# Kr-Stam/CUDA_Optical_Flow_2

Measured on AMD Instinct MI355X. Metric: Mpix/s dense LK flow, higher is better.
Workload: dtype i32/f64; 1 GPU; 3840x2160 pair, 5-level pyramid, 9x9 window, iters=5 (BASELINE.json config as written; iterations = extension lk_iter: bilinear-warp refinement, iteration 1 = the reference bit for bit), mode lk_float, stream path: new frame's pyramid + every LK level and iteration, inputs resident in HBM; SURVEY 8d's smooth texture translating by (2,1) px per frame; warmup_steps_run=5

## Files before the change

### cuda_optical_flow_2_amd/csrc/lk_body_pair.h

```cpp
#pragma once

namespace ofx_dev {

template <int R>
struct TileGeomP {
    static constexpr int FIRST_COL = 2 * R + 2;
    static constexpr int LO_LANE = (FIRST_COL + 3) / 4;
    static constexpr int HI_LANE = 63 - LO_LANE;
    static constexpr int OUT_W = (HI_LANE - LO_LANE + 1) * 4;
    static_assert(4 * LO_LANE >= FIRST_COL && 4 * HI_LANE + 3 <= 253 - 2 * R, "B's output columns have all of A's results they need");
};
static_assert(TileGeomP<4>::LO_LANE == 3 && TileGeomP<4>::HI_LANE == 60 && TileGeomP<4>::OUT_W == 232, "9x9: lanes 3..60");
static_assert(TileGeomP<3>::LO_LANE == 2 && TileGeomP<3>::HI_LANE == 61 && TileGeomP<3>::OUT_W == 240, "7x7: lanes 2..61");
static_assert(TileGeomP<2>::LO_LANE == 2 && TileGeomP<2>::HI_LANE == 61 && TileGeomP<2>::OUT_W == 240, "5x5: lanes 2..61");
static_assert(TileGeomP<1>::LO_LANE == 1 && TileGeomP<1>::HI_LANE == 62 && TileGeomP<1>::OUT_W == 248, "3x3: lanes 1..62");

constexpr int kLkPairMaxR = 4;
constexpr int pair_warp_rows(int r) { return 2 * r + 4; }
constexpr int pair_flow_rows(int r) { return r + 3; }
constexpr int pair_wave_lds(int r) { return kLkWaveLds + 256 * pair_warp_rows(r) + 2048 * pair_flow_rows(r); }
static_assert(pair_wave_lds(4) == 19584 && 8 * pair_wave_lds(4) <= 160 * 1024, "two waves per SIMD at 9x9");

constexpr int pair_seg_steps(int r) { return 3 * r + 4; }

template <int R, bool FAST, bool INTERIOR, bool WOUT>
__device__ __forceinline__ void lk_wave_pair(const LkTable &T, int level, int tile, int ysB, int yeB, int lane, uint8_t *xlds, int q1, int q2, int q3)
{
    constexpr int MODE = OFX_MODE_LK_FLOAT;
    using G = TileGeomP<R>;
    constexpr int NS = 2 * R + 1, H = R - 1, PR = 2 * R - H;
    constexpr int kLagSteps = 2 * R + 3;
    constexpr int WN = pair_warp_rows(R), FN = pair_flow_rows(R);
    static_assert(PR + kLagSteps == pair_seg_steps(R), "a segment of r rows takes r + 3R + 4 steps");

    LkArgs A = T.lv[level];
    pin_scalar(A.w);
    pin_scalar(A.h);
    pin_scalar(A.pitch);
    pin_scalar(A.min_det);
    pin_scalar(A.warp_scale);
    const SolveOpts sopt{A.min_det};
    const int cb = tile * G::OUT_W - G::LO_LANE * 4 + 4 * lane;
    const int ysA = ysB - (R + 1), yeA = min(yeB + R + 1, A.h);

    const int plane_bytes = A.h * A.pitch;
    const __amdgpu_buffer_rsrc_t rs_prev = make_rsrc(A.prev, plane_bytes), rs_next = make_rsrc(A.next, plane_bytes);
    const __amdgpu_buffer_rsrc_t rs_fin = make_rsrc(A.flow_in, A.h * A.w * 8), rs_flow = make_rsrc(A.flow, A.h * A.w * 8);
    const __amdgpu_buffer_rsrc_t rs_wsrc = make_rsrc(A.warp_src, plane_bytes + 3);
    [[maybe_unused]] __amdgpu_buffer_rsrc_t rs_wout = rs_prev;
    if constexpr (WOUT) rs_wout = make_rsrc(A.warp_out, plane_bytes);

    const bool ld_ok = INTERIOR || (cb >= 0 && cb < A.w);
    uint32_t bmask = INTERIOR ? 0xffffffffu : 0u;
    if constexpr (!INTERIOR) {
#pragma unroll
        for (int j = 0; j < 4; ++j) {
            const bool in = (cb + j) >= 0 && (cb + j) < A.w;
            bmask |= in ? (0xffu << (8 * j)) : 0u;
        }
    }
    uint32_t col_off = ld_ok ? (uint32_t)cb : 0u;
    uint32_t nat_off = (uint32_t)cb * 8u;
    auto finish_row = [&](uint32_t raw) -> uint32_t {
        if constexpr (INTERIOR) return raw;
        else return raw & bmask;
    };
    const int x0 = tile * G::OUT_W;
    const int nv = min(x0 + G::OUT_W, A.w) - x0;
    uint32_t l16 = 16u * (uint32_t)lane;
    const int lim = 8 * nv - 16, c16 = 16 * lane;
    const bool st_lo4 = c16 <= lim, st_lo2 = c16 == lim + 8, st_hi4 = c16 <= lim - 1024, st_hi2 = c16 == lim + 8 - 1024;
    const uint32_t vo_lo = st_lo4 ? l16 : (uint32_t)kOob, vo_hi = st_hi4 ? l16 + 1024u : (uint32_t)kOob;
    const bool ragged = __any(st_lo2 || st_hi2) != 0;
    const lds_ptr xl_w = (lds_ptr)xlds + 32 * lane;
    const lds_ptr xl_base = (lds_ptr)xlds + 32 * G::LO_LANE;
    const lds_ptr wring = (lds_ptr)xlds + kLkWaveLds + 4 * lane;
    const lds_ptr fring = (lds_ptr)xlds + kLkWaveLds + 256 * WN + 32 * lane;
    auto wslot = [&](int y) -> int { return __builtin_amdgcn_readfirstlane((int)((uint32_t)(y + 2 * WN) % (uint32_t)WN) * 256); };
    auto fslot = [&](int y) -> int { return __builtin_amdgcn_readfirstlane((int)((uint32_t)(y + 4 * FN) % (uint32_t)FN) * 2048); };
    [[maybe_unused]] uint32_t wvo = (uint32_t)kOob;
    if constexpr (WOUT) {
        const bool out_lane = lane >= G::LO_LANE && lane <= G::HI_LANE && cb < A.w;
        wvo = out_lane ? (uint32_t)cb : (uint32_t)kOob;
    }
    uint32_t wmiss = 0u;
    WarpRowState WA;
    [[maybe_unused]] WarpRowState WB;
    warp_row_clear(WA);
    if constexpr (WOUT) warp_row_clear(WB);
    const s2 two = pk_two();
    const int fstep = A.w * 8;

    const int y_limA = min(yeA + R + 1, A.h);
    const int y_firstA = ysA - R, y_lo0A = y_firstA + H;
    const int nstepsA = (yeA - ysA) + PR;
    const int y_min_outA = max(0, y_firstA - 1), span_outA = max(y_limA - y_min_outA, 0);
    auto row_offA = [&](int y) -> int { return (uint32_t)y < (uint32_t)y_limA ? y * A.pitch : kOob; };
    auto row_off_outA = [&](int y) -> int { return (uint32_t)(y - y_min_outA) < (uint32_t)span_outA ? y * A.pitch : kOob; };
    auto load_u32 = [&](const __amdgpu_buffer_rsrc_t &rs, int po) -> uint32_t { return __builtin_amdgcn_raw_buffer_load_b32(rs, col_off, po, 0); };
    RowPk<MODE> wa[3];
    {
        uint32_t pi, ni, po = 0u, no = 0u;
#pragma unroll
        for (int t = 0; t < 3; ++t) {
            const int oi = row_offA(y_lo0A - 1 + t);
            pi = finish_row(load_u32(rs_prev, oi)), ni = finish_row(load_u32(rs_next, oi));
            if constexpr (H > 0) {
                const int oo = row_off_outA(y_firstA - 1 + t);
                po = finish_row(load_u32(rs_prev, oo)), no = finish_row(load_u32(rs_next, oo));
            }
            unpack_pk(pi, ni, po, no, wa[t]);
        }
    }
    int axx[4] = {0, 0, 0, 0}, ayy[4] = {0, 0, 0, 0}, axy[4] = {0, 0, 0, 0}, axt[4] = {0, 0, 0, 0}, ayt[4] = {0, 0, 0, 0};

    auto ring_warped = [&](int y) {
        const uint32_t wn = finish_row(warp_row_finish(WA));
        *(__attribute__((address_space(3))) uint32_t *)(wring + wslot(y)) = wn;
    };
    auto stepA = [&](auto K, int s) {
        constexpr int k = decltype(K)::value;
        const int yy = y_lo0A + s, yo = yy - NS;
        const bool folded = H > 0 && s < H;
        const int yh = folded ? y_firstA + s : yo;
        const int ro = (H > 1 && s + 1 < H) ? y_firstA + s + 2 : yo + 2;
        const int po_in = row_offA(yy + 2), po_out = row_off_outA(ro);
        const uint32_t pf_ip = load_u32(rs_prev, po_in), pf_in = load_u32(rs_next, po_in);
        const uint32_t pf_op = load_u32(rs_prev, po_out), pf_on = load_u32(rs_next, po_out);
        const bool emit = s >= PR;
        const int yw = yy - R;
        f32x4 old_a, old_b;
        asm("" : "=v"(old_a), "=v"(old_b));
        if (emit) {
            const int fnat = __builtin_amdgcn_readfirstlane(yw >= 0 ? yw * fstep : kOob);
            if constexpr (INTERIOR) {
                old_a = __builtin_bit_cast(f32x4, __builtin_amdgcn_raw_buffer_load_b128(rs_fin, nat_off, fnat, 0));
                old_b = __builtin_bit_cast(f32x4, __builtin_amdgcn_raw_buffer_load_b128(rs_fin, nat_off + 16u, fnat, 0));
            } else {
                auto off = [&](int j) { return ((bmask >> (8 * j)) & 1u) ? nat_off + 8u * (uint32_t)j : (uint32_t)kOob; };
                const u32x2 p0 = __builtin_amdgcn_raw_buffer_load_b64(rs_fin, off(0), fnat, 0), p1 = __builtin_amdgcn_raw_buffer_load_b64(rs_fin, off(1), fnat, 0);
                const u32x2 p2 = __builtin_amdgcn_raw_buffer_load_b64(rs_fin, off(2), fnat, 0), p3 = __builtin_amdgcn_raw_buffer_load_b64(rs_fin, off(3), fnat, 0);
                old_a = __builtin_bit_cast(f32x4, u32x4{p0.x, p0.y, p1.x, p1.y});
                old_b = __builtin_bit_cast(f32x4, u32x4{p2.x, p2.y, p3.x, p3.y});
            }
        }
        const uint32_t him = folded ? 0x00010000u : (yo >= y_firstA ? 0xffff0000u : 0u);
        uint32_t rowm = ((uint32_t)yy < (uint32_t)A.h ? 0x00000001u : 0u) | ((uint32_t)yh < (uint32_t)A.h ? him : 0u);
        if constexpr (INTERIOR) rowm = (uint32_t)__builtin_amdgcn_readfirstlane((int)rowm);
        uint32_t mm[4];
#pragma unroll
        for (int j = 0; j < 4; ++j) mm[j] = INTERIOR ? rowm : ((uint32_t)__builtin_amdgcn_sbfe((int)bmask, 8 * j, 1) & rowm);
        s2 ix[4], iy[4], it[4];
        derivs_pk(wa[k], wa[(k + 1) % 3], wa[(k + 2) % 3], two, ix, iy, it);
        accumulate_pk(ix, iy, it, mm, axx, ayy, axy, axt, ayt);
        if (emit) {
            float uv[8];
            int hb[5][4];
            {
                int va[5][4];
#pragma unroll
                for (int j = 0; j < 4; ++j) va[0][j] = axx[j], va[1][j] = ayy[j], va[2][j] = axy[j], va[3][j] = axt[j], va[4][j] = ayt[j];
                hbox4x5<R>(va, hb);
            }
            solve_lane<MODE, FAST>(hb[0], hb[1], hb[2], hb[3], hb[4], sopt, uv);
            uv[0] = old_a.x + uv[0], uv[1] = old_a.y + uv[1], uv[2] = old_a.z + uv[2], uv[3] = old_a.w + uv[3];
            uv[4] = old_b.x + uv[4], uv[5] = old_b.y + uv[5], uv[6] = old_b.z + uv[6], uv[7] = old_b.w + uv[7];
            ring_warped(yw - 1);
            const float fu[4] = {uv[0], uv[2], uv[4], uv[6]}, fv[4] = {uv[1], uv[3], uv[5], uv[7]};
            warp_row_prepare<false>(rs_wsrc, A.warp_scale, A.w, A.h, A.pitch, 0, A.h, cb, yw, 4, fu, fv, WA, wmiss);
            const lds_ptr fr = fring + fslot(yw);
            *(__attribute__((address_space(3))) f32x4 *)(fr) = f32x4{uv[0], uv[1], uv[2], uv[3]};
            *(__attribute__((address_space(3))) f32x4 *)(fr + 16) = f32x4{uv[4], uv[5], uv[6], uv[7]};
        }
        unpack_pk(finish_row(pf_ip), finish_row(pf_in), finish_row(pf_op), finish_row(pf_on), wa[k]);
        pin_row(wa[k]);
    };

    const int y_limB = min(yeB + R + 1, A.h);
    const int y_firstB = ysB - R, y_lo0B = y_firstB + H;
    const int nstepsB = (yeB - ysB) + PR;
    const int y_min_outB = max(0, y_firstB - 1), span_outB = max(y_limB - y_min_outB, 0);
    auto row_offB = [&](int y) -> int { return (uint32_t)y < (uint32_t)y_limB ? y * A.pitch : kOob; };
    auto row_off_outB = [&](int y) -> int { return (uint32_t)(y - y_min_outB) < (uint32_t)span_outB ? y * A.pitch : kOob; };
    auto ring_row = [&](int y, int po) -> uint32_t {
        uint32_t v = 0u;
        if (po != kOob) v = *(const __attribute__((address_space(3))) uint32_t *)(wring + wslot(y));
        return v;
    };
    RowPk<MODE> wb[3];
    uint32_t pfb_i = 0u, pfb_o = 0u;
    int bxx[4] = {0, 0, 0, 0}, byy[4] = {0, 0, 0, 0}, bxy[4] = {0, 0, 0, 0}, bxt[4] = {0, 0, 0, 0}, byt[4] = {0, 0, 0, 0};
    const int fso0 = __builtin_amdgcn_readfirstlane((ysB * A.w + x0) * 8);
    auto high_rowB = [&](int s) -> int { return (H > 0 && (s == 0 || s < H)) ? y_firstB + s + 1 : y_lo0B + s - NS + 1; };
    auto primeB = [&]() {
        uint32_t pi, ni, po = 0u, no = 0u;
#pragma unroll
        for (int t = 0; t < 2; ++t) {
            const int yi = y_lo0B - 1 + t, oi = row_offB(yi);
            pi = finish_row(load_u32(rs_prev, oi)), ni = ring_row(yi, oi);
            if constexpr (H > 0) {
                const int yo = y_firstB - 1 + t, oo = row_off_outB(yo);
                po = finish_row(load_u32(rs_prev, oo)), no = ring_row(yo, oo);
            }
            unpack_pk(pi, ni, po, no, wb[t]);
        }
        pfb_i = load_u32(rs_prev, row_offB(y_lo0B + 1));
        pfb_o = load_u32(rs_prev, H > 0 ? row_off_outB(high_rowB(0)) : kOob);
    };
    auto store_row = [&](int s_row, const f32x4 xlo, const f32x4 xhi) {
        const int fso = __builtin_amdgcn_readfirstlane(fso0 + (s_row - PR) * fstep);
        __builtin_amdgcn_raw_buffer_store_b128(__builtin_bit_cast(u32x4, xlo), rs_flow, INTERIOR ? lane_off_var(l16) : vo_lo, fso, kLkStoreAux);
        __builtin_amdgcn_raw_buffer_store_b128(__builtin_bit_cast(u32x4, xhi), rs_flow, vo_hi, fso, kLkStoreAux);
        if (__builtin_expect(ragged, 0)) {
            const u32x4 ql = __builtin_bit_cast(u32x4, xlo), qh = __builtin_bit_cast(u32x4, xhi);
            __builtin_amdgcn_raw_buffer_store_b64(u32x2{ql.x, ql.y}, rs_flow, st_lo2 ? l16 : (uint32_t)kOob, fso, kLkStoreAux);
            __builtin_amdgcn_raw_buffer_store_b64(u32x2{qh.x, qh.y}, rs_flow, st_hi2 ? l16 + 1024u : (uint32_t)kOob, fso, kLkStoreAux);
        }
    };
    auto stepB = [&](auto K, int s) {
        constexpr int k = decltype(K)::value;
        const int yy = y_lo0B + s, yo = yy - NS;
        const bool folded = H > 0 && s < H;
        const int yh = folded ? y_firstB + s : yo;
        {
            const int rh = high_rowB(s);
            const int oi = row_offB(yy + 1), oo = (H > 0 || s > 0) ? row_off_outB(rh) : kOob;
            unpack_pk(finish_row(pfb_i), ring_row(yy + 1, oi), finish_row(pfb_o), ring_row(rh, oo), wb[(k + 2) % 3]);
            pin_row(wb[(k + 2) % 3]);
            pfb_i = load_u32(rs_prev, row_offB(yy + 2));
            pfb_o = load_u32(rs_prev, row_off_outB(high_rowB(s + 1)));
        }
        const bool emit = s >= PR;
        const int yw = yy - R;
        f32x4 old_a, old_b;
        asm("" : "=v"(old_a), "=v"(old_b));
        if (emit) {
            const lds_ptr fr = fring + fslot(yw);
            old_a = *(const __attribute__((address_space(3))) f32x4 *)(fr);
            old_b = *(const __attribute__((address_space(3))) f32x4 *)(fr + 16);
        }
        const uint32_t him = folded ? 0x00010000u : (yo >= y_firstB ? 0xffff0000u : 0u);
        uint32_t rowm = ((uint32_t)yy < (uint32_t)A.h ? 0x00000001u : 0u) | ((uint32_t)yh < (uint32_t)A.h ? him : 0u);
        if constexpr (INTERIOR) rowm = (uint32_t)__builtin_amdgcn_readfirstlane((int)rowm);
        uint32_t mm[4];
#pragma unroll
        for (int j = 0; j < 4; ++j) mm[j] = INTERIOR ? rowm : ((uint32_t)__builtin_amdgcn_sbfe((int)bmask, 8 * j, 1) & rowm);
        s2 ix[4], iy[4], it[4];
        derivs_pk(wb[k], wb[(k + 1) % 3], wb[(k + 2) % 3], two, ix, iy, it);
        accumulate_pk(ix, iy, it, mm, bxx, byy, bxy, bxt, byt);
        if (emit) {
            float uv[8];
            int hb[5][4];
            {
                int va[5][4];
#pragma unroll
                for (int j = 0; j < 4; ++j) va[0][j] = bxx[j], va[1][j] = byy[j], va[2][j] = bxy[j], va[3][j] = bxt[j], va[4][j] = byt[j];
                hbox4x5<R>(va, hb);
            }
            solve_lane<MODE, FAST>(hb[0], hb[1], hb[2], hb[3], hb[4], sopt, uv);
            uv[0] = old_a.x + uv[0], uv[1] = old_a.y + uv[1], uv[2] = old_a.z + uv[2], uv[3] = old_a.w + uv[3];
            uv[4] = old_b.x + uv[4], uv[5] = old_b.y + uv[5], uv[6] = old_b.z + uv[6], uv[7] = old_b.w + uv[7];
            if constexpr (WOUT) {
                const uint32_t wn = warp_row_finish(WB);
                const int wso = __builtin_amdgcn_readfirstlane(s > PR ? (yw - 1) * A.pitch : kOob);
                __builtin_amdgcn_raw_buffer_store_b32(wn, rs_wout, wvo, wso, 0);
                const float fu[4] = {uv[0], uv[2], uv[4], uv[6]}, fv[4] = {uv[1], uv[3], uv[5], uv[7]};
                warp_row_prepare<false>(rs_wsrc, A.warp_scale, A.w, A.h, A.pitch, 0, A.h, cb, yw, 4, fu, fv, WB, wmiss);
            }
            *(__attribute__((address_space(3))) f32x4 *)(xl_w) = f32x4{uv[0], uv[1], uv[2], uv[3]};
            *(__attribute__((address_space(3))) f32x4 *)(xl_w + 16) = f32x4{uv[4], uv[5], uv[6], uv[7]};
            __builtin_amdgcn_fence(__ATOMIC_SEQ_CST, "wavefront");
            __builtin_amdgcn_wave_barrier();
            const lds_ptr xl_r = xl_base + lane_off_var(l16);
            const f32x4 xlo = *(__attribute__((address_space(3))) f32x4 *)(xl_r);
            const f32x4 xhi = *(__attribute__((address_space(3))) f32x4 *)(xl_r + 1024);
            store_row(s, xlo, xhi);
        }
    };

    const int nsteps = nstepsB + kLagSteps;
    auto body = [&](auto K, int t) {
        constexpr int k = decltype(K)::value;
        constexpr int kb = (k + 3 - kLagSteps % 3) % 3;
        if (t < nstepsA) stepA(K, t);
        else if (t == nstepsA) ring_warped(yeA - 1);
        if (t >= kLagSteps) {
            __builtin_amdgcn_fence(__ATOMIC_SEQ_CST, "wavefront");
            __builtin_amdgcn_wave_barrier();
            if constexpr (kb == 0) {
                if (t == kLagSteps) primeB();
            }
            stepB(std::integral_constant<int, kb>{}, t - kLagSteps);
        }
    };
    int s = 0;
    while (true) {
        body(std::integral_constant<int, 0>{}, s);
        if (++s >= nsteps) break;
        body(std::integral_constant<int, 1>{}, s);
        if (++s >= nsteps) break;
        body(std::integral_constant<int, 2>{}, s);
        if (++s >= nsteps) break;
        OFX_LK_PRIO_STEP();
    }
    if constexpr (WOUT) {
        const uint32_t wn = warp_row_finish(WB);
        __builtin_amdgcn_raw_buffer_store_b32(wn, rs_wout, wvo, (yeB - 1) * A.pitch, 0);
    }
}

}
```

### cuda_optical_flow_2_amd/csrc/lk_solve.h

```cpp
#pragma once

#include <hip/hip_runtime.h>

#include "ofx.h"

__device__ __forceinline__ double recip_f64(double x)
{
    double p = __builtin_amdgcn_rcp(x);
    double e = __builtin_fma(-x, p, 1.0);
    const double t = __builtin_fma(e, e, e);
    p = __builtin_fma(p, t, p);
    e = __builtin_fma(-x, p, 1.0);
    p = __builtin_fma(p, e, p);
    return __builtin_amdgcn_div_fixup(p, x, 1.0);
}

struct SolveOpts {
    float min_det;
};

template <int MODE>
__device__ __forceinline__ void solve_tail_exact(double a, double b, double d, double xt, double yt, double det, float &u, float &v)
{
    const double pre = recip_f64(det);
    double c = b;
    a *= pre;
    b *= pre;
    if constexpr (MODE == OFX_MODE_LK_FLOAT) c *= pre;
    d *= pre;
    u = (float)(-d * xt + b * yt);
    v = (float)(c * xt - a * yt);
}

template <int MODE>
__device__ __forceinline__ void solve_operands(int sxx, int syy, int sxy, int sxt, int syt, double &a, double &b, double &d, double &xt,
                                               double &yt, double &det)
{
    if constexpr (MODE == OFX_MODE_LK_FLOAT) {
        a = (double)(float)sxx;
        b = (double)(float)sxy;
        d = (double)(float)syy;
        xt = (double)(float)sxt;
        yt = (double)(float)syt;
        det = __builtin_fma(a, d, -(b * b));
    } else {
        a = (double)sxx;
        b = (double)sxy;
        d = (double)syy;
        xt = (double)sxt;
        yt = (double)syt;
        det = a * d - b * b;
    }
}

__device__ __forceinline__ unsigned long long solve_fast(int sxx, int syy, int sxy, int sxt, int syt, float &u, float &v)
{
    double a, b, d, xt, yt, det;
    solve_operands<OFX_MODE_LK_FLOAT>(sxx, syy, sxy, sxt, syt, a, b, d, xt, yt, det);
    const double nu = __builtin_fma(b, yt, -(d * xt));
    const double nv = __builtin_fma(b, xt, -(a * yt));
    double p = __builtin_amdgcn_rcp(det);
    const double e = __builtin_fma(-det, p, 1.0);
    p = __builtin_fma(p, e, p);
    u = (float)(nu * p);
    v = (float)(nv * p);
    return __ballot(det == 0.0);
}

__device__ __forceinline__ void solve_fix_singular(int sxx, int syy, int sxy, int sxt, int syt, float &u, float &v)
{
    double a, b, d, xt, yt, det;
    solve_operands<OFX_MODE_LK_FLOAT>(sxx, syy, sxy, sxt, syt, a, b, d, xt, yt, det);
    float eu, ev;
    solve_tail_exact<OFX_MODE_LK_FLOAT>(a, b, d, xt, yt, det, eu, ev);
    if (det == 0.0) {
        u = eu;
        v = ev;
    }
}

template <int MODE>
__device__ __forceinline__ void solve_guard(int sxx, int syy, int sxy, float min_det, float &u, float &v)
{
    double a, b, d, xt, yt, det;
    solve_operands<MODE>(sxx, syy, sxy, 0, 0, a, b, d, xt, yt, det);
    if (!((float)det >= min_det)) {
        u = 0.0f;
        v = 0.0f;
    }
}

template <int MODE, bool FAST>
__device__ __forceinline__ void solve2x2(int sxx, int syy, int sxy, int sxt, int syt, const SolveOpts &opt, float &u, float &v)
{
    static_assert(!FAST || MODE == OFX_MODE_LK_FLOAT, "the fast solve is defined for lk_float only");
    if constexpr (FAST) {
        if (solve_fast(sxx, syy, sxy, sxt, syt, u, v) != 0ull) solve_fix_singular(sxx, syy, sxy, sxt, syt, u, v);
    } else {
        double a, b, d, xt, yt, det;
        solve_operands<MODE>(sxx, syy, sxy, sxt, syt, a, b, d, xt, yt, det);
        solve_tail_exact<MODE>(a, b, d, xt, yt, det, u, v);
    }
    if (__builtin_expect(opt.min_det > 0.0f, 0)) {
        asm volatile("" : "+v"(u), "+v"(v));
        solve_guard<MODE>(sxx, syy, sxy, opt.min_det, u, v);
    }
}

template <int MODE, bool FAST>
__device__ __forceinline__ void solve_lane(const int (&sxx)[4], const int (&syy)[4], const int (&sxy)[4], const int (&sxt)[4],
                                           const int (&syt)[4], const SolveOpts &opt, float (&uv)[8])
{
    if constexpr (FAST) {
#pragma unroll
        for (int j = 0; j < 4; ++j) {
            if (__builtin_expect(solve_fast(sxx[j], syy[j], sxy[j], sxt[j], syt[j], uv[2 * j], uv[2 * j + 1]) != 0ull, 0)) {
                asm volatile("" : "+v"(uv[2 * j]), "+v"(uv[2 * j + 1]));
                solve_fix_singular(sxx[j], syy[j], sxy[j], sxt[j], syt[j], uv[2 * j], uv[2 * j + 1]);
            }
        }
    } else {
#pragma unroll
        for (int j = 0; j < 4; ++j) {
            double a, b, d, xt, yt, det;
            solve_operands<MODE>(sxx[j], syy[j], sxy[j], sxt[j], syt[j], a, b, d, xt, yt, det);
            solve_tail_exact<MODE>(a, b, d, xt, yt, det, uv[2 * j], uv[2 * j + 1]);
        }
    }
    if (__builtin_expect(opt.min_det > 0.0f, 0)) {
        asm volatile("" : "+v"(uv[0]), "+v"(uv[1]), "+v"(uv[2]), "+v"(uv[3]), "+v"(uv[4]), "+v"(uv[5]), "+v"(uv[6]), "+v"(uv[7]));
#pragma unroll
        for (int j = 0; j < 4; ++j) solve_guard<MODE>(sxx[j], syy[j], sxy[j], opt.min_det, uv[2 * j], uv[2 * j + 1]);
    }
}
```

Measured before the change: 34970 Mpix/s.

## Share the determinant reciprocal from pass A with pass B through a register delay queue

In the paired-pass LK kernel, the structure-tensor determinant for an output row is the same in both passes, because it depends only on spatial gradients. Pass A now exports its per-lane f64 reciprocal of det, and pass B consumes it after a register delay queue that matches B's lag behind A. This removes pass B's f64 rcp and Newton refinement. In exchange it keeps about two dozen extra doubles live in VGPRs, which may cost occupancy or cause spills at the two-waves-per-SIMD target. Pass B's singular fallback is now detected as a NaN reciprocal instead of det == 0.

```diff
diff --git a/cuda_optical_flow_2_amd/csrc/lk_body_pair.h b/cuda_optical_flow_2_amd/csrc/lk_body_pair.h
--- a/cuda_optical_flow_2_amd/csrc/lk_body_pair.h
+++ b/cuda_optical_flow_2_amd/csrc/lk_body_pair.h
@@ -15,6 +15,11 @@
 static_assert(TileGeomP<2>::LO_LANE == 2 && TileGeomP<2>::HI_LANE == 61 && TileGeomP<2>::OUT_W == 240, "5x5: lanes 2..61");
 static_assert(TileGeomP<1>::LO_LANE == 1 && TileGeomP<1>::HI_LANE == 62 && TileGeomP<1>::OUT_W == 248, "3x3: lanes 1..62");
 
+#ifndef OFX_PAIR_SHARE_RCP
+#define OFX_PAIR_SHARE_RCP 1
+#endif
+constexpr bool pair_share_rcp(int r, bool fast) { return OFX_PAIR_SHARE_RCP != 0; }
+
 constexpr int kLkPairMaxR = 4;
 constexpr int pair_warp_rows(int r) { return 2 * r + 4; }
 constexpr int pair_flow_rows(int r) { return r + 3; }
@@ -32,6 +37,16 @@
     constexpr int kLagSteps = 2 * R + 3;
     constexpr int WN = pair_warp_rows(R), FN = pair_flow_rows(R);
     static_assert(PR + kLagSteps == pair_seg_steps(R), "a segment of r rows takes r + 3R + 4 steps");
+    constexpr bool SHARE = pair_share_rcp(R, FAST);
+    constexpr int QD = (R + 2) / 3, QE = (R + 2) % 3;
+    static_assert(QD >= 1 && 3 * QD + QE == kLagSteps - (R + 1), "the delay is B's lag behind A on an output row");
+    [[maybe_unused]] double rq[QD][3][4], rc[QE > 0 ? QE : 1][4];
+    if constexpr (SHARE) {
+#pragma unroll
+        for (int i = 0; i < QD * 3; ++i) asm volatile("" : "=v"(rq[i / 3][i % 3][0]), "=v"(rq[i / 3][i % 3][1]), "=v"(rq[i / 3][i % 3][2]), "=v"(rq[i / 3][i % 3][3]));
+#pragma unroll
+        for (int i = 0; i < QE; ++i) asm volatile("" : "=v"(rc[i][0]), "=v"(rc[i][1]), "=v"(rc[i][2]), "=v"(rc[i][3]));
+    }
 
     LkArgs A = T.lv[level];
     pin_scalar(A.w);
@@ -114,6 +129,9 @@
     }
     int axx[4] = {0, 0, 0, 0}, ayy[4] = {0, 0, 0, 0}, axy[4] = {0, 0, 0, 0}, axt[4] = {0, 0, 0, 0}, ayt[4] = {0, 0, 0, 0};
 
+    auto no_rcp = [](double (&q)[4]) {
+        if constexpr (SHARE) asm("" : "=v"(q[0]), "=v"(q[1]), "=v"(q[2]), "=v"(q[3]));
+    };
     auto ring_warped = [&](int y) {
         const uint32_t wn = finish_row(warp_row_finish(WA));
         *(__attribute__((address_space(3))) uint32_t *)(wring + wslot(y)) = wn;
@@ -162,7 +180,8 @@
                 for (int j = 0; j < 4; ++j) va[0][j] = axx[j], va[1][j] = ayy[j], va[2][j] = axy[j], va[3][j] = axt[j], va[4][j] = ayt[j];
                 hbox4x5<R>(va, hb);
             }
-            solve_lane<MODE, FAST>(hb[0], hb[1], hb[2], hb[3], hb[4], sopt, uv);
+            if constexpr (SHARE) solve_lane_rcp_out<MODE, FAST>(hb[0], hb[1], hb[2], hb[3], hb[4], sopt, rq[0][k], uv);
+            else solve_lane<MODE, FAST>(hb[0], hb[1], hb[2], hb[3], hb[4], sopt, uv);
             uv[0] = old_a.x + uv[0], uv[1] = old_a.y + uv[1], uv[2] = old_a.z + uv[2], uv[3] = old_a.w + uv[3];
             uv[4] = old_b.x + uv[4], uv[5] = old_b.y + uv[5], uv[6] = old_b.z + uv[6], uv[7] = old_b.w + uv[7];
             ring_warped(yw - 1);
@@ -171,7 +190,7 @@
             const lds_ptr fr = fring + fslot(yw);
             *(__attribute__((address_space(3))) f32x4 *)(fr) = f32x4{uv[0], uv[1], uv[2], uv[3]};
             *(__attribute__((address_space(3))) f32x4 *)(fr + 16) = f32x4{uv[4], uv[5], uv[6], uv[7]};
-        }
+        } else no_rcp(rq[0][k]);
         unpack_pk(finish_row(pf_ip), finish_row(pf_in), finish_row(pf_op), finish_row(pf_on), wa[k]);
         pin_row(wa[k]);
     };
@@ -217,7 +236,7 @@
             __builtin_amdgcn_raw_buffer_store_b64(u32x2{qh.x, qh.y}, rs_flow, st_hi2 ? l16 + 1024u : (uint32_t)kOob, fso, kLkStoreAux);
         }
     };
-    auto stepB = [&](auto K, int s) {
+    auto stepB = [&](auto K, int s, [[maybe_unused]] const double (&rcp)[4]) {
         constexpr int k = decltype(K)::value;
         const int yy = y_lo0B + s, yo = yy - NS;
         const bool folded = H > 0 && s < H;
@@ -257,7 +276,8 @@
                 for (int j = 0; j < 4; ++j) va[0][j] = bxx[j], va[1][j] = byy[j], va[2][j] = bxy[j], va[3][j] = bxt[j], va[4][j] = byt[j];
                 hbox4x5<R>(va, hb);
             }
-            solve_lane<MODE, FAST>(hb[0], hb[1], hb[2], hb[3], hb[4], sopt, uv);
+            if constexpr (SHARE) solve_lane_rcp_in<MODE, FAST>(hb[0], hb[1], hb[2], hb[3], hb[4], sopt, rcp, uv);
+            else solve_lane<MODE, FAST>(hb[0], hb[1], hb[2], hb[3], hb[4], sopt, uv);
             uv[0] = old_a.x + uv[0], uv[1] = old_a.y + uv[1], uv[2] = old_a.z + uv[2], uv[3] = old_a.w + uv[3];
             uv[4] = old_b.x + uv[4], uv[5] = old_b.y + uv[5], uv[6] = old_b.z + uv[6], uv[7] = old_b.w + uv[7];
             if constexpr (WOUT) {
@@ -282,15 +302,31 @@
     auto body = [&](auto K, int t) {
         constexpr int k = decltype(K)::value;
         constexpr int kb = (k + 3 - kLagSteps % 3) % 3;
+        [[maybe_unused]] double rcpB[4];
+        if constexpr (SHARE) {
+#pragma unroll
+            for (int j = 0; j < 4; ++j) {
+                const double out = rq[QD - 1][k][j];
+                rcpB[j] = QE > 0 ? rc[QE > 0 ? QE - 1 : 0][j] : out;
+#pragma unroll
+                for (int i = QE - 1; i > 0; --i) rc[i][j] = rc[i - 1][j];
+                if constexpr (QE > 0) rc[0][j] = out;
+#pragma unroll
+                for (int i = QD - 1; i > 0; --i) rq[i][k][j] = rq[i - 1][k][j];
+            }
+        }
         if (t < nstepsA) stepA(K, t);
-        else if (t == nstepsA) ring_warped(yeA - 1);
+        else {
+            if (t == nstepsA) ring_warped(yeA - 1);
+            no_rcp(rq[0][k]);
+        }
         if (t >= kLagSteps) {
             __builtin_amdgcn_fence(__ATOMIC_SEQ_CST, "wavefront");
             __builtin_amdgcn_wave_barrier();
             if constexpr (kb == 0) {
                 if (t == kLagSteps) primeB();
             }
-            stepB(std::integral_constant<int, kb>{}, t - kLagSteps);
+            stepB(std::integral_constant<int, kb>{}, t - kLagSteps, rcpB);
         }
     };
     int s = 0;
diff --git a/cuda_optical_flow_2_amd/csrc/lk_solve.h b/cuda_optical_flow_2_amd/csrc/lk_solve.h
--- a/cuda_optical_flow_2_amd/csrc/lk_solve.h
+++ b/cuda_optical_flow_2_amd/csrc/lk_solve.h
@@ -20,9 +20,8 @@
 };
 
 template <int MODE>
-__device__ __forceinline__ void solve_tail_exact(double a, double b, double d, double xt, double yt, double det, float &u, float &v)
+__device__ __forceinline__ void solve_tail_pre(double a, double b, double d, double xt, double yt, double pre, float &u, float &v)
 {
-    const double pre = recip_f64(det);
     double c = b;
     a *= pre;
     b *= pre;
@@ -30,6 +29,12 @@
     d *= pre;
     u = (float)(-d * xt + b * yt);
     v = (float)(c * xt - a * yt);
+}
+
+template <int MODE>
+__device__ __forceinline__ void solve_tail_exact(double a, double b, double d, double xt, double yt, double det, float &u, float &v)
+{
+    solve_tail_pre<MODE>(a, b, d, xt, yt, recip_f64(det), u, v);
 }
 
 template <int MODE>
@@ -53,18 +58,30 @@
     }
 }
 
-__device__ __forceinline__ unsigned long long solve_fast(int sxx, int syy, int sxy, int sxt, int syt, float &u, float &v)
+enum { kRcpOwn = 0, kRcpOut = 1, kRcpIn = 2 };
+
+template <int RCP>
+__device__ __forceinline__ unsigned long long solve_fast_rcp(int sxx, int syy, int sxy, int sxt, int syt, double &p, float &u, float &v)
 {
     double a, b, d, xt, yt, det;
     solve_operands<OFX_MODE_LK_FLOAT>(sxx, syy, sxy, sxt, syt, a, b, d, xt, yt, det);
     const double nu = __builtin_fma(b, yt, -(d * xt));
     const double nv = __builtin_fma(b, xt, -(a * yt));
-    double p = __builtin_amdgcn_rcp(det);
-    const double e = __builtin_fma(-det, p, 1.0);
-    p = __builtin_fma(p, e, p);
+    if constexpr (RCP != kRcpIn) {
+        p = __builtin_amdgcn_rcp(det);
+        const double e = __builtin_fma(-det, p, 1.0);
+        p = __builtin_fma(p, e, p);
+    }
     u = (float)(nu * p);
     v = (float)(nv * p);
-    return __ballot(det == 0.0);
+    if constexpr (RCP == kRcpIn) return __ballot(p != p);
+    else return __ballot(det == 0.0);
+}
+
+__device__ __forceinline__ unsigned long long solve_fast(int sxx, int syy, int sxy, int sxt, int syt, float &u, float &v)
+{
+    double p;
+    return solve_fast_rcp<kRcpOwn>(sxx, syy, sxy, sxt, syt, p, u, v);
 }
 
 __device__ __forceinline__ void solve_fix_singular(int sxx, int syy, int sxy, int sxt, int syt, float &u, float &v)
@@ -107,14 +124,14 @@
     }
 }
 
-template <int MODE, bool FAST>
-__device__ __forceinline__ void solve_lane(const int (&sxx)[4], const int (&syy)[4], const int (&sxy)[4], const int (&sxt)[4],
-                                           const int (&syt)[4], const SolveOpts &opt, float (&uv)[8])
+template <int MODE, bool FAST, int RCP>
+__device__ __forceinline__ void solve_lane_rcp(const int (&sxx)[4], const int (&syy)[4], const int (&sxy)[4], const int (&sxt)[4],
+                                               const int (&syt)[4], const SolveOpts &opt, double (&rcp)[4], float (&uv)[8])
 {
     if constexpr (FAST) {
 #pragma unroll
         for (int j = 0; j < 4; ++j) {
-            if (__builtin_expect(solve_fast(sxx[j], syy[j], sxy[j], sxt[j], syt[j], uv[2 * j], uv[2 * j + 1]) != 0ull, 0)) {
+            if (__builtin_expect(solve_fast_rcp<RCP>(sxx[j], syy[j], sxy[j], sxt[j], syt[j], rcp[j], uv[2 * j], uv[2 * j + 1]) != 0ull, 0)) {
                 asm volatile("" : "+v"(uv[2 * j]), "+v"(uv[2 * j + 1]));
                 solve_fix_singular(sxx[j], syy[j], sxy[j], sxt[j], syt[j], uv[2 * j], uv[2 * j + 1]);
             }
@@ -124,7 +141,8 @@
         for (int j = 0; j < 4; ++j) {
             double a, b, d, xt, yt, det;
             solve_operands<MODE>(sxx[j], syy[j], sxy[j], sxt[j], syt[j], a, b, d, xt, yt, det);
-            solve_tail_exact<MODE>(a, b, d, xt, yt, det, uv[2 * j], uv[2 * j + 1]);
+            if constexpr (RCP != kRcpIn) rcp[j] = recip_f64(det);
+            solve_tail_pre<MODE>(a, b, d, xt, yt, rcp[j], uv[2 * j], uv[2 * j + 1]);
         }
     }
     if (__builtin_expect(opt.min_det > 0.0f, 0)) {
@@ -133,3 +151,26 @@
         for (int j = 0; j < 4; ++j) solve_guard<MODE>(sxx[j], syy[j], sxy[j], opt.min_det, uv[2 * j], uv[2 * j + 1]);
     }
 }
+
+template <int MODE, bool FAST>
+__device__ __forceinline__ void solve_lane(const int (&sxx)[4], const int (&syy)[4], const int (&sxy)[4], const int (&sxt)[4],
+                                           const int (&syt)[4], const SolveOpts &opt, float (&uv)[8])
+{
+    double rcp[4];
+    solve_lane_rcp<MODE, FAST, kRcpOwn>(sxx, syy, sxy, sxt, syt, opt, rcp, uv);
+}
+
+template <int MODE, bool FAST>
+__device__ __forceinline__ void solve_lane_rcp_out(const int (&sxx)[4], const int (&syy)[4], const int (&sxy)[4], const int (&sxt)[4],
+                                                   const int (&syt)[4], const SolveOpts &opt, double (&rcp)[4], float (&uv)[8])
+{
+    solve_lane_rcp<MODE, FAST, kRcpOut>(sxx, syy, sxy, sxt, syt, opt, rcp, uv);
+}
+
+template <int MODE, bool FAST>
+__device__ __forceinline__ void solve_lane_rcp_in(const int (&sxx)[4], const int (&syy)[4], const int (&sxy)[4], const int (&sxt)[4],
+                                                  const int (&syt)[4], const SolveOpts &opt, const double (&rcp)[4], float (&uv)[8])
+{
+    double r[4] = {rcp[0], rcp[1], rcp[2], rcp[3]};
+    solve_lane_rcp<MODE, FAST, kRcpIn>(sxx, syy, sxy, sxt, syt, opt, r, uv);
+}
```

New measurement: 35780 Mpix/s (median of 6 runs). +2.3%, better.
